# CoHDI/composable-resource-operator

Hardware: AMD Instinct MI355X
Metric: p50 GPU attach→CDI-ready latency (ms) + reconciles/sec at 1/2/4/8 MI355X (lower is better)
Workload: dtype bf16; 1 GPU; model=ComposabilityRequest(type=gpu, model=mi355x, size=1) bulk compose, global_batch=1, seq_len=0, fabric=mock (in-process; no physical CXL fabric on bench node), probe=True, force_detach=False, cpus=4, gc_frozen=True

## Files before the change

cro_amd/controllers/composableresource.py:

```python

from __future__ import annotations

import logging
import time
from dataclasses import dataclass
from typing import Dict, Optional

from ..api.v1alpha1.types import ComposableResource
from ..fabric import Adapter, FabricError, WaitingDeviceAttaching, WaitingDeviceDetaching
from ..metrics import Metrics
from ..nodeops import amdgpu, taints
from ..nodeops.amdgpu import GPULoadsPresent, ScrubFailed
from ..nodeops.nodes import node_exists
from ..runtime.client import Client
from ..runtime.controller import Reconciler, Result
from ..runtime.errors import ConflictError, NotFoundError
from ..runtime.store import _now_rfc3339

log = logging.getLogger(__name__)

FINALIZER = "cro.amd.com/finalizer"
READY_TO_DETACH_LABEL = "cro.amd.com/ready-to-detach-device-id"
READY_TO_DETACH_CDI_LABEL = "cro.amd.com/ready-to-detach-cdi-device-id"
MANAGED_BY_LABEL = "app.kubernetes.io/managed-by"
# ... 313 lines not shown
            for other in self.client.list(ComposableResource, copy=False):
                if (
                    other.metadata.name != resource.metadata.name
                    and other.status.device_id == device_id
                ):
                    raise FabricError(
                        f"fabric returned device {device_id} already claimed "
                        f"by {other.metadata.name}; refusing dual attachment"
                    )
            resource = self._persist_device_identity(
                resource.metadata.name, device_id, cdi_device_id
            )
            self._fabric_polls.pop(resource.metadata.uid, None)
            self.recorder.normal(
                resource, "FabricAttached", f"fabric composed device {device_id}"
            )

        if mode == "DEVICE_PLUGIN":
            try:
                ops.check_no_loads(node)
            except GPULoadsPresent as exc:
                log.warning("gpu loads during attach on %s: %s", node, exc)
            resource = self._restart_plugin_daemonsets(resource, fatal=False)
        with self._phase("node_refresh"):
            ops.refresh_after_attach(node)

        if mode == "DRA":
            visible = ops.is_visible_dra(node, resource.status.device_id)
        else:
            visible = ops.is_visible(node, resource.status.device_id)
        if not visible:
            return Result(requeue_after=self.config.attach_visible_wait)

        with self._phase("cdi_write"):
            ops.write_cdi(node, resource.status.device_id)
        with self._phase("health_probe"):
            probe = ops.health_probe(node, resource.status.device_id)
        if probe is not None and not probe.get("ok", True):
            compute = probe.get("compute")
            if isinstance(compute, dict) and not compute.get("ok", True):
                test = compute.get("failed_test") or (
                    "coverage" if compute.get("rc") == -31 else "unknown"
                )
                self.metrics.probe_compute_failures_total.labels(test=test).inc()
                raise FabricError(
                    "gfx950 health probe failed: compute stage "
# ... 239 lines not shown
```

cro_amd/hip/build.py:

```python

from __future__ import annotations

import os
import subprocess
import sys

HIP_DIR = os.path.dirname(os.path.abspath(__file__))
AGENT_DIR = os.path.join(os.path.dirname(HIP_DIR), "agent")
SRC = os.path.join(HIP_DIR, "probe.hip")
SRCS = [SRC, os.path.join(HIP_DIR, "integrity.hip")]
HEADERS = [os.path.join(HIP_DIR, "croprobe.h"), os.path.join(HIP_DIR, "cropattern.h")]
COVERAGE_SRC = os.path.join(HIP_DIR, "coverage.hip")
COVERAGE_HEADER = os.path.join(HIP_DIR, "crocoverage.h")
INTERNAL_HEADERS = [os.path.join(HIP_DIR, "crohost.h"), os.path.join(HIP_DIR, "cromfma.h")]
INTEGRITY_HEADER = os.path.join(HIP_DIR, "crointegrity.h")
ALL_SRCS = SRCS + [COVERAGE_SRC]
ALL_HEADERS = HEADERS + [COVERAGE_HEADER, INTEGRITY_HEADER] + INTERNAL_HEADERS
OUT = os.path.join(HIP_DIR, "libcroprobe.so")
SCRUB_SRC = os.path.join(HIP_DIR, "scrub.hip")
SCRUB_HEADERS = [
    os.path.join(HIP_DIR, "croscrub.h"),
    os.path.join(HIP_DIR, "croscrubplan.h"),
    os.path.join(HIP_DIR, "crohost.h"),
    INTEGRITY_HEADER,
    HEADERS[1],
]
SCRUB_OUT = os.path.join(HIP_DIR, "libcroscrub.so")
LDS_SCRUB_SRC = os.path.join(HIP_DIR, "ldsscrub.hip")
LDS_SCRUB_HEADERS = [
    os.path.join(HIP_DIR, "croldsscrub.h"),
    os.path.join(HIP_DIR, "crohost.h"),
    COVERAGE_HEADER,
]
LDS_SCRUB_OUT = os.path.join(HIP_DIR, "libcroldsscrub.so")
REG_SCRUB_SRC = os.path.join(HIP_DIR, "regscrub.hip")
REG_SCRUB_HEADERS = [
    os.path.join(HIP_DIR, "croregscrub.h"),
    os.path.join(HIP_DIR, "crohost.h"),
    COVERAGE_HEADER,
]
# ... 14 lines not shown
]
COHERENCE_OUT = os.path.join(HIP_DIR, "libcrocoherence.so")
MOVEMENT_SRC = os.path.join(HIP_DIR, "movement.hip")
MOVEMENT_HEADERS = [
    os.path.join(HIP_DIR, "cromovement.h"),
    os.path.join(HIP_DIR, "crohost.h"),
    COVERAGE_HEADER,
]
MOVEMENT_OUT = os.path.join(HIP_DIR, "libcromovement.so")
AGENT_SRC = os.path.join(AGENT_DIR, "croagent.cpp")
AGENT_OUT = os.path.join(AGENT_DIR, "croagent")
HIPCC = os.environ.get("HIPCC", "/opt/rocm/bin/hipcc")
DEVICE_FLAGS = ["--offload-arch=gfx950", "-O3"]


def _stale(out: str, inputs) -> bool:
    if not os.path.exists(out):
        return True
    built = os.path.getmtime(out)
    return any(os.path.getmtime(path) > built for path in inputs)


def build(force: bool = False) -> str:
    if force or _stale(OUT, ALL_SRCS + ALL_HEADERS):
        subprocess.run(
            [HIPCC, *DEVICE_FLAGS, "-fPIC", "-shared", *ALL_SRCS, "-o", OUT],
            check=True,
        )
    build_agent(force=force)
    return OUT


def build_scrub(force: bool = False) -> str:
    if force or _stale(SCRUB_OUT, [SCRUB_SRC] + SCRUB_HEADERS):
        subprocess.run(
            [HIPCC, *DEVICE_FLAGS, "-fPIC", "-shared", SCRUB_SRC, "-o", SCRUB_OUT],
            check=True,
        )
    return SCRUB_OUT


def build_lds_scrub(force: bool = False) -> str:
    if force or _stale(LDS_SCRUB_OUT, [LDS_SCRUB_SRC] + LDS_SCRUB_HEADERS):
        subprocess.run(
            [HIPCC, *DEVICE_FLAGS, "-fPIC", "-shared", LDS_SCRUB_SRC, "-o", LDS_SCRUB_OUT],
            check=True,
        )
# ... 71 lines not shown
```

cro_amd/hip/croprobe.h:

```cpp
#pragma once

#include "crocoverage.h"

#ifdef __cplusplus
extern "C" {
#endif

struct CroProbeResult {
  int ok;
  int mfma_f32_exact;
  double hbm_gbps;
  double bf16_tflops;
  long long vram_total;
  long long vram_free;
  double t_setup_ms;
  double t_mfma_ms;
  double t_bw_ms;
  double t_bf16_ms;
  char gcn_arch[64];
  char msg[256];
};

struct CroProbeOpts {
  double hbm_floor_gbps;
  double bf16_floor_tflops;
  int selftest_mode;
  int selftest_bit;
  unsigned int selftest_elem;
  int reserved;
};

int cro_probe_run(int device, struct CroProbeResult* out);
int cro_probe_run_opts(int device, const struct CroProbeOpts* opts, struct CroProbeResult* out);

struct CroProbeWindows {
  int copy_launches;
  int bf16_iters;
  int skip_check_launch;
  int reserved;
};

int cro_probe_run_windows(int device, const struct CroProbeWindows* w,
                          struct CroProbeResult* out);
int cro_probe_mfma_f32(int device, const float* A, const float* B, float* D, int K);
int cro_probe_copy(int device, const void* src_host, unsigned long long n4, int grid_blocks,
                   void* dst_host, int* guard_ok);
int cro_probe_bw_selfcheck(int device, unsigned long long* n_bad,
                           unsigned long long* first_bad);
int cro_probe_bf16_sink(int device, int blocks, int iters, int all_lanes, float* out_host);
void* cro_probe_alloc(int device, long long bytes);
void cro_probe_free(void* p);
int cro_probe_device_count(void);
int cro_probe_pci_bus_id(int device, char* buf, int len);


struct CroIntegrityOpts {
  long long vram_bytes;
  long long link_bytes;
  long long chunk_bytes;
  unsigned int seed;
  int selftest_stage;
  double link_floor_gbps;
  int selftest_pass;
  int selftest_bit;
  unsigned long long selftest_word;
};
// ... 99 lines not shown
```

cro_amd/hip/probe.hip:

```cpp

#include <hip/hip_runtime.h>
#include <hip/hip_bf16.h>
#include <cstring>
#include <vector>

#include "crohost.h"
#include "cromfma.h"
#include "croprobe.h"


__global__ void mfma_f32_check_kernel(const float* __restrict__ A,
                                      const float* __restrict__ B,
                                      float* __restrict__ D, int K) {
  const uint32_t lane = threadIdx.x;
  const f32x4 acc = wave_mfma_f32(A, B, K, lane);
  for (int r = 0; r < 4; ++r) D[mfma_elem16(lane, r)] = acc[r];
}


__global__ void bw_copy_kernel(const float4* __restrict__ src,
                               float4* __restrict__ dst, size_t n4) {
  size_t i = (size_t)blockIdx.x * blockDim.x + threadIdx.x;
  size_t stride = (size_t)gridDim.x * blockDim.x;
  for (; i < n4; i += stride) dst[i] = src[i];
}


template <bool kAllLanes>
__global__ void mfma_bf16_rate_kernel(float* __restrict__ out, int iters) {
  bf16x8 a, b;
  for (int i = 0; i < 8; ++i) {
// ... 9 lines not shown
  }
  float s = 0.f;
  for (int i = 0; i < 16; ++i) s += acc0[i] + acc1[i] + acc2[i] + acc3[i];
  if constexpr (kAllLanes) {
    out[blockIdx.x * 256 + threadIdx.x] = s;
  } else {
    if (threadIdx.x == 0) out[blockIdx.x] = s;
  }
}


enum { kEvCheck0, kEvCheck1, kEvCopies, kEvRate, kEvTile, kNumEvents };

struct ProbeCtx : CtxBase {
  long long vram_total = 0, vram_free = 0;
  float *dA = nullptr, *dB = nullptr, *dD = nullptr;
  float4 *src = nullptr, *dst = nullptr;
  float* sink = nullptr;
  hipStream_t stream = nullptr;
  hipEvent_t ev[kNumEvents] = {};
  float* hD = nullptr;
  float refD[CRO_COV_F32_ELEMS] = {0};
  char gcn_arch[64] = {0};
};
static ProbeCtx g_ctx[kMaxDevices];

constexpr int kBwGrid = 8192;
constexpr size_t kBwBytes = (size_t)256 << 20;
constexpr int kGuardVecs = 64;
constexpr unsigned long long kMaxCopyVecs = kBwBytes / sizeof(float4);
constexpr int kMaxCopyGrid = 1 << 16;
constexpr int kMaxSinkBlocks = 1024;
constexpr int kMaxSinkIters = 1 << 16;
constexpr int kRateBlocks = 1024;
constexpr int kDefaultCopyLaunches = 8;
constexpr int kDefaultBf16Iters = 1024;
constexpr int kMaxCopyLaunches = 64;
constexpr int kMaxBf16Iters = 1 << 16;

static void launch_copy(const float4* src, float4* dst, size_t n4, int grid_blocks,
                        hipStream_t stream = nullptr) {
  hipLaunchKernelGGL(bw_copy_kernel, dim3(grid_blocks), dim3(kBlock), 0, stream, src, dst, n4);
}

static void launch_probe_copy(const ProbeCtx* ctx) {
  launch_copy(ctx->src, ctx->dst, kBwBytes / sizeof(float4), kBwGrid, ctx->stream);
// ... 34 lines not shown
  ctx->vram_total = (long long)total_b;
  ctx->vram_free = (long long)free_b;
  TRY(hipDeviceSynchronize());
  TRY(hipMemsetAsync(ctx->dD, 0xFF, sizeof(ctx->refD), ctx->stream));
  launch_probe_check(ctx);
  launch_probe_copy(ctx);
  launch_probe_rate(ctx, 64);
  TRY(hipGetLastError());
  TRY(hipMemcpyAsync(ctx->hD, ctx->dD, sizeof(ctx->refD), hipMemcpyDeviceToHost, ctx->stream));
  TRY(hipStreamSynchronize(ctx->stream));
  ctx->ready = 1;
  return hipSuccess;
}

#define STEP(expr)                \
  do {                            \
    hipError_t _e = (expr);       \
    if (_e != hipSuccess) {       \
      *what = #expr;              \
      return _e;                  \
    }                             \
  } while (0)

static hipError_t enqueue_and_wait(ProbeCtx* ctx, int copy_launches, int bf16_iters,
                                   bool skip_check, bool* enqueued, const char** what) {
  hipStream_t st = ctx->stream;
  *enqueued = true;
  STEP(hipMemsetAsync(ctx->dD, 0xFF, sizeof(ctx->refD), st));
  STEP(hipEventRecord(ctx->ev[kEvCheck0], st));
  if (!skip_check) launch_probe_check(ctx);
  STEP(hipGetLastError());
  STEP(hipEventRecord(ctx->ev[kEvCheck1], st));
  for (int i = 0; i < copy_launches; ++i) launch_probe_copy(ctx);
  STEP(hipGetLastError());
  STEP(hipEventRecord(ctx->ev[kEvCopies], st));
  launch_probe_rate(ctx, bf16_iters);
  STEP(hipGetLastError());
  STEP(hipEventRecord(ctx->ev[kEvRate], st));
  STEP(hipMemcpyAsync(ctx->hD, ctx->dD, sizeof(ctx->refD), hipMemcpyDeviceToHost, st));
  STEP(hipEventRecord(ctx->ev[kEvTile], st));
  STEP(hipEventSynchronize(ctx->ev[kEvTile]));
  return hipSuccess;
}

#undef STEP

static int run_pipeline(int device, const struct CroProbeOpts& o, int copy_launches,
                        int bf16_iters, bool skip_check, struct CroProbeResult* out, double t0) {
  const double hbm_floor = o.hbm_floor_gbps > 0.0 ? o.hbm_floor_gbps : 500.0;
  const double bf16_floor = o.bf16_floor_tflops > 0.0 ? o.bf16_floor_tflops : 100.0;

  std::unique_lock<std::mutex> lock;
  ProbeCtx* ctx = enter_device(g_ctx, device, lock, out->msg, sizeof(out->msg));
  if (ctx == nullptr) return -1;
  CHECK(ensure_ctx(ctx, device));
  snprintf(out->gcn_arch, sizeof(out->gcn_arch), "%s", ctx->gcn_arch);
  out->vram_total = ctx->vram_total;
  out->vram_free = ctx->vram_free;
  out->t_setup_ms = now_ms() - t0;

  bool enqueued = false;
  const char* what = "";
  const hipError_t e = enqueue_and_wait(ctx, copy_launches, bf16_iters, skip_check, &enqueued,
                                        &what);
  if (e != hipSuccess) {
    if (enqueued) (void)hipStreamSynchronize(ctx->stream);
    snprintf(out->msg, sizeof(out->msg), "%s failed: %s", what, hipGetErrorString(e));
    return -1;
  }

  const float* want = ctx->refD;
  float flipped[CRO_COV_F32_ELEMS];
  if (o.selftest_mode == 1) {
    memcpy(flipped, ctx->refD, sizeof(flipped));
    uint32_t u;
    memcpy(&u, &flipped[o.selftest_elem], sizeof(u));
    u ^= 1u << o.selftest_bit;
    memcpy(&flipped[o.selftest_elem], &u, sizeof(u));
    want = flipped;
  }
  out->mfma_f32_exact = (memcmp(ctx->hD, want, sizeof(flipped)) == 0) ? 1 : 0;

  float ms = 0.f;
  CHECK(hipEventElapsedTime(&ms, ctx->ev[kEvCheck0], ctx->ev[kEvCheck1]));
  out->t_mfma_ms = ms;
  CHECK(hipEventElapsedTime(&ms, ctx->ev[kEvCheck1], ctx->ev[kEvCopies]));
  out->hbm_gbps = (double)(2.0 * kBwBytes * copy_launches) / (ms * 1e6);
  out->t_bw_ms = ms;
  CHECK(hipEventElapsedTime(&ms, ctx->ev[kEvCopies], ctx->ev[kEvRate]));
  double waves = (double)kRateBlocks * 256.0 / 64.0;
  double flops = waves * 4.0 * (double)bf16_iters * 2.0 * 32.0 * 32.0 * 16.0;
  out->bf16_tflops = flops / (ms * 1e9);
  out->t_bf16_ms = ms;

  if (!out->mfma_f32_exact) {
    snprintf(out->msg, sizeof(out->msg), "f32 MFMA mismatch vs host fmaf chain");
    return -2;
  }
  if (out->hbm_gbps < hbm_floor) {
    snprintf(out->msg, sizeof(out->msg), "HBM bandwidth %.0f GB/s below floor", out->hbm_gbps);
    return -3;
  }
  if (out->bf16_tflops < bf16_floor) {
    snprintf(out->msg, sizeof(out->msg), "bf16 MFMA %.0f TF below floor", out->bf16_tflops);
    return -4;
  }
  out->ok = 1;
  snprintf(out->msg, sizeof(out->msg), "ok");
  return 0;
}

extern "C" int cro_probe_run_opts(int device, const struct CroProbeOpts* opts,
                                  struct CroProbeResult* out) {
  memset(out, 0, sizeof(*out));
  out->ok = 0;
  const double t0 = now_ms();

  struct CroProbeOpts o;
  memset(&o, 0, sizeof(o));
  if (opts) o = *opts;
  if (!(o.hbm_floor_gbps >= 0.0)) return bad_arg(out, "hbm_floor_gbps");
  if (!(o.bf16_floor_tflops >= 0.0)) return bad_arg(out, "bf16_floor_tflops");
  if (o.selftest_mode < 0 || o.selftest_mode > 1) return bad_arg(out, "selftest_mode");
  if (o.selftest_bit < 0 || o.selftest_bit > 31) return bad_arg(out, "selftest_bit");
  if (o.selftest_elem >= CRO_COV_F32_ELEMS) return bad_arg(out, "selftest_elem");
  return run_pipeline(device, o, kDefaultCopyLaunches, kDefaultBf16Iters, false, out, t0);
}

extern "C" int cro_probe_run_windows(int device, const struct CroProbeWindows* w,
                                     struct CroProbeResult* out) {
  memset(out, 0, sizeof(*out));
  out->ok = 0;
  const double t0 = now_ms();

  struct CroProbeWindows win;
  memset(&win, 0, sizeof(win));
  if (w) win = *w;
  if (win.copy_launches < 0 || win.copy_launches > kMaxCopyLaunches)
    return bad_arg(out, "copy_launches");
  if (win.bf16_iters < 0 || win.bf16_iters > kMaxBf16Iters) return bad_arg(out, "bf16_iters");
  if (win.skip_check_launch < 0 || win.skip_check_launch > 1)
    return bad_arg(out, "skip_check_launch");
  if (win.reserved < 0) return bad_arg(out, "reserved");
  struct CroProbeOpts o;
  memset(&o, 0, sizeof(o));
  return run_pipeline(device, o, win.copy_launches ? win.copy_launches : kDefaultCopyLaunches,
                      win.bf16_iters ? win.bf16_iters : kDefaultBf16Iters,
                      win.skip_check_launch == 1, out, t0);
}

extern "C" int cro_probe_run(int device, struct CroProbeResult* out) {
  return cro_probe_run_opts(device, nullptr, out);
}


extern "C" int cro_probe_mfma_f32(int device, const float* A, const float* B,
                                  float* D, int K) {
  if (A == nullptr || B == nullptr || D == nullptr) return -10;
  if (K <= 0 || K > kMaxTileK || (K & 3) != 0) return -10;
  const size_t in_bytes = (size_t)16 * K * sizeof(float), out_bytes = 256 * sizeof(float);
  if (hipSetDevice(device) != hipSuccess) return -1;
  DevBuf<float> dA, dB, dD;
  const auto run = [&]() -> hipError_t {
    TRY(dA.alloc(in_bytes));
    TRY(dB.alloc(in_bytes));
    TRY(dD.alloc(out_bytes));
    TRY(hipMemcpy(dA.get(), A, in_bytes, hipMemcpyHostToDevice));
    TRY(hipMemcpy(dB.get(), B, in_bytes, hipMemcpyHostToDevice));
    hipLaunchKernelGGL(mfma_f32_check_kernel, dim3(1), dim3(64), 0, 0, dA.get(), dB.get(),
                       dD.get(), K);
    TRY(hipGetLastError());
// ... 19 lines not shown
    TRY(hipMemcpy(src.get(), src_host, bytes, hipMemcpyHostToDevice));
    TRY(hipMemset(dst.get(), 0xA5, bytes + guard_bytes));
    launch_copy(src.get(), dst.get(), (size_t)n4, grid_blocks);
    TRY(hipGetLastError());
    TRY(hipMemcpy(dst_host, dst.get(), bytes, hipMemcpyDeviceToHost));
    TRY(hipMemcpy(back.data(), dst.get() + n4, guard_bytes, hipMemcpyDeviceToHost));
    int ok = 1;
    for (size_t i = 0; i < guard_bytes; ++i) ok &= back[i] == 0xA5;
    *guard_ok = ok;
    return hipMemcpy(back.data(), src.get(), bytes, hipMemcpyDeviceToHost);
  };
  if (run() != hipSuccess) return -1;
  return memcmp(back.data(), src_host, bytes) == 0 ? 0 : -11;
}

extern "C" int cro_probe_bw_selfcheck(int device, unsigned long long* n_bad,
                                      unsigned long long* first_bad) {
  if (n_bad == nullptr || first_bad == nullptr) return -10;
  *n_bad = 0;
  *first_bad = ~0ull;
  std::unique_lock<std::mutex> lock;
  ProbeCtx* ctx = enter_device(g_ctx, device, lock, nullptr, 0);
  if (ctx == nullptr) return -1;
  const auto copy_once = [&]() -> hipError_t {
    TRY(ensure_ctx(ctx, device));
    TRY(hipMemsetAsync(ctx->dst, 0, kBwBytes, ctx->stream));
    launch_probe_copy(ctx);
    TRY(hipGetLastError());
    return hipSuccess;
  };
  const hipError_t enq = copy_once();
  const hipError_t done = ctx->stream ? hipStreamSynchronize(ctx->stream) : hipSuccess;
  if (enq != hipSuccess || done != hipSuccess) return -1;
  const size_t chunk = (size_t)32 << 20;
  std::vector<unsigned char> host(chunk);
  for (size_t off = 0; off < kBwBytes; off += chunk) {
    if (hipMemcpy(host.data(), (const unsigned char*)ctx->dst + off, chunk,
                  hipMemcpyDeviceToHost) != hipSuccess)
      return -1;
    for (size_t i = 0; i < chunk; i += 8) {
      unsigned long long w;
      memcpy(&w, &host[i], 8);
      if (w == 0x5a5a5a5a5a5a5a5aull) continue;
      for (size_t j = i; j < i + 8; ++j) {
        if (host[j] == 0x5a) continue;
        if (*n_bad == 0) *first_bad = off + j;
// ... 52 lines not shown
```

cro_amd/nodeops/amdgpu.py:

```python

from __future__ import annotations

import logging
import threading
import time
from typing import Callable, Dict, List, Optional, Set

from ..api.v1alpha1.types import ResourceSlice, ResourceSliceDevice, ResourceSliceSpec
from .cdi_spec import CDISpecWriter
from .execs import ExecError, NodeExec
from .kfd import GPUDevice, enumerate_gpus, enumerate_gpus_amdsmi, gpu_compute_pids

log = logging.getLogger(__name__)


class DriverMissing(Exception):
    pass


class GPULoadsPresent(Exception):
    pass


class ScrubFailed(Exception):
# ... 18 lines not shown

    def is_visible(self, node: str, device_id: str) -> bool:
        raise NotImplementedError

    def check_no_loads(self, node: str, device_id: Optional[str] = None) -> None:
        raise NotImplementedError

    def drain(self, node: str, device_id: str) -> None:
        raise NotImplementedError

    def refresh_after_attach(self, node: str) -> None:
        raise NotImplementedError

    def refresh_after_detach(self, node: str) -> None:
        raise NotImplementedError

    def write_cdi(self, node: str, device_id: str) -> str:
        raise NotImplementedError

    def remove_cdi(self, node: str, device_id: str) -> None:
        raise NotImplementedError

    def health_probe(self, node: str, device_id: str) -> Optional[dict]:
        return None

    def scrub(self, node: str, device_id: str) -> Optional[dict]:
        return None


class AmdNodeOps(NodeOps):
    def __init__(
        self,
        execer: NodeExec,
        client=None,
        cdi_dir: str = "/etc/cdi",
        destructive: bool = True,
        initially_detached: Optional[List[str]] = None,
        restart_hooks: Optional[Dict[str, Callable[[str], None]]] = None,
        probe_fn: Optional[Callable[[int], dict]] = None,
        publish_resource_slices: bool = True,
        scrub_fn: Optional[Callable[[GPUDevice], dict]] = None,
    ):
        self.execer = execer
        self.client = client
        self.cdi = CDISpecWriter(execer, cdi_dir)
        self.destructive = destructive
        self.publish_slices = publish_resource_slices
        self._sim_detached: Set[str] = set(initially_detached or [])
        self._sim_lock = threading.Lock()
        self.restart_hooks = restart_hooks or {}
        self.probe_fn = probe_fn
        self.scrub_fn = scrub_fn
        self._self_pid_cache: Dict[int, Optional[int]] = {}
        self._drain_lock = threading.Lock()
        self._drain_threads: Dict[str, threading.Thread] = {}
        self._drain_errors: Dict[str, str] = {}
        self.enum_cache_ttl = 0.025
        self._enum_cache: Dict[str, tuple] = {}
        self._enum_lock = threading.Lock()
        self._static_meta: dict = {}


    def driver_mode(self, node: str) -> str:
        if self.client is not None:
            from ..api.v1alpha1.types import DeviceConfig

            try:
                configs = self.client.list(DeviceConfig)
            except Exception:
                configs = []
            if any(dc.spec.driver.enable for dc in configs):
                return "container"
        if self.execer.path_exists(node, "/sys/module/amdgpu"):
            return "host"
        return "none"
# ... 149 lines not shown
            if cached is None and gpu_id not in self._self_pid_cache:
                hip_dev = None
                try:
                    from .probe import hip_device_for_bdf, load_library

                    if load_library(required=False) is not None:
                        for g in self.enumerate(node):
                            if g.gpu_id == gpu_id:
                                hip_dev = hip_device_for_bdf(g.pci_bdf)
                                break
                        if hip_dev is not None:
                            cached = resolve_self_kfd_pid(
                                self.execer, node, gpu_id, hip_dev
                            )
                except Exception as exc:
                    log.debug("self-pid resolution failed: %s", exc)
                self._self_pid_cache[gpu_id] = cached
            if cached is not None:
                own.add(cached)
        return own


    def drain(self, node: str, device_id: str) -> None:
        with self._drain_lock:
            thread = self._drain_threads.get(device_id)
            if thread is not None:
                if thread.is_alive():
                    raise DrainInProgress(f"drain of {device_id} still running")
                del self._drain_threads[device_id]
                err = self._drain_errors.pop(device_id, None)
                if err is not None:
                    raise ExecError(err)
                return

        gpu = self.find_gpu(node, device_id)
        if gpu is None:
            return
        if not self.destructive:
            with self._sim_lock:
                self._sim_detached.add(device_id)
            self._invalidate_enum(node)
            return
        remaining = [g for g in self.enumerate(node) if g.device_id != device_id]
        if remaining:
            self.execer.write_file(node, f"/sys/bus/pci/devices/{gpu.pci_bdf}/remove", "1")
            self._invalidate_enum(node)
# ... 4 lines not shown
        def unload_and_remove():
            try:
                rc, _, err = self.execer.run(node, modprobe_argv, timeout=120)
                if rc != 0:
                    raise ExecError(f"modprobe -r amdgpu failed: {err}", rc=rc, stderr=err)
                self.execer.write_file(
                    node, f"/sys/bus/pci/devices/{gpu.pci_bdf}/remove", "1"
                )
                self._invalidate_enum(node)
            except Exception as exc:
                with self._drain_lock:
                    self._drain_errors[device_id] = str(exc)

        t = threading.Thread(target=unload_and_remove, name=f"drain-{device_id}", daemon=True)
        with self._drain_lock:
            self._drain_threads[device_id] = t
        t.start()
        raise DrainInProgress(f"last-device drain of {device_id} started")

    def refresh_after_attach(self, node: str) -> None:
        if self.destructive:
            self.execer.write_file(node, "/sys/bus/pci/rescan", "1")
        self._invalidate_enum(node)
        for name, hook in self.restart_hooks.items():
            try:
                hook(node)
            except Exception as exc:
                log.warning("restart hook %s failed on %s: %s", name, node, exc)
        self._publish_slice(node)

    def simulate_compose(self, node: str, device_id: str) -> None:
        with self._sim_lock:
            self._sim_detached.discard(device_id)
        self._invalidate_enum(node)

    def refresh_after_detach(self, node: str) -> None:
        for name, hook in self.restart_hooks.items():
            try:
                hook(node)
            except Exception as exc:
                log.warning("restart hook %s failed on %s: %s", name, node, exc)
        self._publish_slice(node)

    def _publish_slice(self, node: str) -> None:
        if self.client is None or not self.publish_slices:
            return
        devices = [
            ResourceSliceDevice(
                name=f"gpu-{i}",
                uuid=g.device_id,
                model="mi355x",
                node=node,
# ... 13 lines not shown
            sl.spec = ResourceSliceSpec(node_name=node, pool=name, devices=devices)
            self.client.create(sl)
        else:
            existing.spec.devices = devices
            self.client.update(existing)


    def write_cdi(self, node: str, device_id: str) -> str:
        gpu = self.find_gpu(node, device_id)
        if gpu is None:
            raise ExecError(f"device {device_id} not enumerable; cannot write CDI spec")
        return self.cdi.add_device(node, gpu)

    def remove_cdi(self, node: str, device_id: str) -> None:
        self.cdi.remove_device(node, device_id)


    def health_probe(self, node: str, device_id: str) -> Optional[dict]:
        if self.probe_fn is None:
            return None
        gpu = self.find_gpu(node, device_id)
        if gpu is None:
            return None
        return self.probe_fn(gpu)

    def scrub(self, node: str, device_id: str) -> Optional[dict]:
        if self.scrub_fn is None:
            return None
        gpu = self.find_gpu(node, device_id)
        if gpu is None:
            return None
        return self.scrub_fn(gpu)


class MockNodeOps(NodeOps):

    def __init__(self, client=None, attach_visible_delay: float = 0.0):
        self.client = client
        self.driver_present: Dict[str, bool] = {}
        self.composed: Dict[str, Set[str]] = {}
        self.visible: Dict[str, Set[str]] = {}
        self.loads: Dict[str, Set[str]] = {}
        self.cdi_written: Dict[str, Set[str]] = {}
        from collections import deque

        self.calls: "deque[tuple]" = deque(maxlen=10000)
# ... 83 lines not shown
```

cro_amd/nodeops/probe.py:

```python

from __future__ import annotations

import ctypes
import os
from typing import Optional

_LIB_PATH = os.path.join(os.path.dirname(__file__), "..", "hip", "libcroprobe.so")


class CroProbeResult(ctypes.Structure):
    _fields_ = [
        ("ok", ctypes.c_int),
        ("mfma_f32_exact", ctypes.c_int),
        ("hbm_gbps", ctypes.c_double),
        ("bf16_tflops", ctypes.c_double),
        ("vram_total", ctypes.c_longlong),
        ("vram_free", ctypes.c_longlong),
        ("t_setup_ms", ctypes.c_double),
        ("t_mfma_ms", ctypes.c_double),
        ("t_bw_ms", ctypes.c_double),
        ("t_bf16_ms", ctypes.c_double),
        ("gcn_arch", ctypes.c_char * 64),
        ("msg", ctypes.c_char * 256),
    ]


class CroProbeOpts(ctypes.Structure):

# ... 156 lines not shown
    if _lib is not None:
        return _lib
    if required is None:
        required = _gpu_present()
    path = os.path.abspath(_LIB_PATH)
    if not os.path.exists(path):
        if required:
            raise RuntimeError(
                f"libcroprobe.so missing at {path} on a GPU node — build it with "
                "`python -m cro_amd.hip.build` (hipcc --offload-arch=gfx950)"
            )
        return None
    lib = ctypes.CDLL(path)
    lib.cro_probe_run.argtypes = [ctypes.c_int, ctypes.POINTER(CroProbeResult)]
    lib.cro_probe_run.restype = ctypes.c_int
    lib.cro_probe_run_opts.argtypes = [
        ctypes.c_int, ctypes.POINTER(CroProbeOpts), ctypes.POINTER(CroProbeResult),
    ]
    lib.cro_probe_run_opts.restype = ctypes.c_int
    lib.cro_probe_run_windows.argtypes = [
        ctypes.c_int, ctypes.POINTER(CroProbeWindows), ctypes.POINTER(CroProbeResult),
    ]
    lib.cro_probe_run_windows.restype = ctypes.c_int
    f32p = ctypes.POINTER(ctypes.c_float)
    lib.cro_probe_mfma_f32.argtypes = [ctypes.c_int, f32p, f32p, f32p, ctypes.c_int]
    lib.cro_probe_mfma_f32.restype = ctypes.c_int
    lib.cro_probe_copy.argtypes = [
        ctypes.c_int, ctypes.c_void_p, ctypes.c_ulonglong, ctypes.c_int, ctypes.c_void_p,
        ctypes.POINTER(ctypes.c_int),
    ]
    lib.cro_probe_copy.restype = ctypes.c_int
    lib.cro_probe_bw_selfcheck.argtypes = [
        ctypes.c_int, ctypes.POINTER(ctypes.c_ulonglong), ctypes.POINTER(ctypes.c_ulonglong),
    ]
    lib.cro_probe_bw_selfcheck.restype = ctypes.c_int
    lib.cro_probe_bf16_sink.argtypes = [
        ctypes.c_int, ctypes.c_int, ctypes.c_int, ctypes.c_int, ctypes.c_void_p,
    ]
    lib.cro_probe_bf16_sink.restype = ctypes.c_int
    lib.cro_probe_device_count.restype = ctypes.c_int
    lib.cro_probe_pci_bus_id.argtypes = [ctypes.c_int, ctypes.c_char_p, ctypes.c_int]
    lib.cro_probe_pci_bus_id.restype = ctypes.c_int
    lib.cro_probe_alloc.argtypes = [ctypes.c_int, ctypes.c_longlong]
    lib.cro_probe_alloc.restype = ctypes.c_void_p
    lib.cro_probe_free.argtypes = [ctypes.c_void_p]
    lib.cro_probe_free.restype = None
    lib.cro_probe_integrity.argtypes = [
# ... 107 lines not shown
def run_probe(device: int = 0, **opts) -> dict:
    lib = load_library(required=True)
    res = CroProbeResult()
    if opts:
        c_opts = _probe_opts(**opts)
        rc = lib.cro_probe_run_opts(device, ctypes.byref(c_opts), ctypes.byref(res))
    else:
        rc = lib.cro_probe_run(device, ctypes.byref(res))
    return _result_dict(res, rc)


def run_probe_windows(device: int = 0, copy_launches: int = 0, bf16_iters: int = 0,
                      skip_check_launch: int = 0) -> dict:
    lib = load_library(required=True)
    windows = CroProbeWindows(
        copy_launches=int(copy_launches), bf16_iters=int(bf16_iters),
        skip_check_launch=int(skip_check_launch),
    )
    res = CroProbeResult()
    rc = lib.cro_probe_run_windows(device, ctypes.byref(windows), ctypes.byref(res))
    return _result_dict(res, rc)


def probe_fn_for_nodeops(gpu) -> dict:
    dev = hip_device_for_bdf(gpu.pci_bdf)
    if dev is None:
        dev = 0
    return run_probe(dev)




def mfma_f32_tile(device: int, a, b):
    import numpy as np

    lib = load_library(required=True)
    a = np.ascontiguousarray(a, dtype=np.float32)
    b = np.ascontiguousarray(b, dtype=np.float32)
    k = a.shape[1] if a.ndim == 2 else -1
    if a.shape != (16, k) or b.shape != (k, 16):
        raise ValueError("f32 tile wants A 16xK and B Kx16")
    d = np.zeros((16, 16), dtype=np.float32)
    f32p = ctypes.POINTER(ctypes.c_float)
    rc = lib.cro_probe_mfma_f32(device, a.ctypes.data_as(f32p), b.ctypes.data_as(f32p),
                                d.ctypes.data_as(f32p), k)
    if rc != 0:
        raise RuntimeError(f"cro_probe_mfma_f32 failed: rc={rc}")
    return d


def copy_vectors(device: int, words, grid_blocks: int) -> dict:
# ... 409 lines not shown


def aggregate_records(records) -> dict:
    out, _, bad_keys = aggregate_wave_records(records, ("f32", "i8", "bf16", "lds"))
    out.update(n_bad_cu_keys=min(len(bad_keys), 8), bad_cu_keys=bad_keys[:8])
    return out


def make_probe_fn(level: str = "quick", vram_bytes: int = 0, link_bytes: int = 0,
                  link_floor_gbps: float = 0.0, seed: int = 0, compute: bool = False,
                  compute_min_cu_fraction: float = 0.0, formats: bool = False,
                  formats_min_cu_fraction: float = 0.0, coherence: bool = False,
                  coherence_min_cu_fraction: float = 0.0, movement: bool = False,
                  movement_min_cu_fraction: float = 0.0):
    if level not in PROBE_LEVELS:
        raise ValueError(f"unknown probe level {level!r} (expected one of {PROBE_LEVELS})")
    if level == "quick" and not compute and not formats and not coherence and not movement:
        return probe_fn_for_nodeops

    def staged_probe(gpu) -> dict:
        dev = hip_device_for_bdf(gpu.pci_bdf)
        if dev is None:
            dev = 0
        result = run_probe(dev)
        if not result.get("ok"):
            return result
        if compute:
            stage = run_compute(dev, seed=seed, min_cu_fraction=compute_min_cu_fraction)
            result["compute"] = stage
            if not stage.get("ok"):
                result["ok"] = False
                result["msg"] = stage.get("msg", "compute probe failed")
                return result
        if formats:
            from .formats import run_formats

            stage = run_formats(dev, seed=seed, min_cu_fraction=formats_min_cu_fraction)
            result["formats"] = stage
            if not stage.get("ok"):
                result["ok"] = False
                result["msg"] = stage.get("msg", "formats probe failed")
                return result
        if coherence:
            from .coherence import run_coherence

            stage = run_coherence(dev, seed=seed, min_cu_fraction=coherence_min_cu_fraction)
            result["coherence"] = stage
# ... 2 lines not shown
                result["msg"] = stage.get("msg", "coherence probe failed")
                return result
        if movement:
            from .movement import run_movement

            stage = run_movement(dev, seed=seed, min_cu_fraction=movement_min_cu_fraction)
            result["movement"] = stage
            if not stage.get("ok"):
                result["ok"] = False
                result["msg"] = stage.get("msg", "movement probe failed")
                return result
        if level == "deep":
            integrity = run_integrity(
                dev, vram_bytes=vram_bytes, link_bytes=link_bytes, seed=seed,
                link_floor_gbps=link_floor_gbps,
            )
            result["integrity"] = integrity
            if not integrity.get("ok"):
                result["ok"] = False
                result["msg"] = integrity.get("msg", "integrity probe failed")
        return result

    staged_probe.level = level
    staged_probe.compute = bool(compute)
    if formats:
        staged_probe.formats = True
    if coherence:
        staged_probe.coherence = True
    if movement:
        staged_probe.movement = True
    return staged_probe


def _compute_argv(compute, compute_min_cu_fraction) -> list:
    if not compute:
        return []
    argv = ["--compute"]
    if compute_min_cu_fraction:
        argv += ["--compute-min-cu-fraction", str(float(compute_min_cu_fraction))]
    return argv


def _formats_argv(formats, formats_min_cu_fraction) -> list:
    if not formats:
        return []
    argv = ["--formats"]
# ... 87 lines not shown
```

Baseline: 3.124 ms.

## Split GPU health probe into async submit/collect to overlap with node refresh

Adds a ticketed submit/collect/cancel API to the HIP probe library so the probe pipeline can be enqueued without waiting on its completion event. The controller now requests a probe before node refresh, nodeops submits it right after enumeration invalidation, and the later health_probe call collects the in-flight result instead of launching and synchronizing from scratch. This is meant to hide GPU probe execution behind node refresh, CDI write and the visibility check, at the cost of ticket bookkeeping, cancellation on drain, and a fallback to a synchronous run if the ticket is stale.

```diff
diff --git a/cro_amd/controllers/composableresource.py b/cro_amd/controllers/composableresource.py
--- a/cro_amd/controllers/composableresource.py
+++ b/cro_amd/controllers/composableresource.py
@@ -359,6 +359,9 @@
             except GPULoadsPresent as exc:
                 log.warning("gpu loads during attach on %s: %s", node, exc)
             resource = self._restart_plugin_daemonsets(resource, fatal=False)
+        begin_probe = getattr(ops, "begin_health_probe", None)
+        if begin_probe is not None:
+            begin_probe(node, resource.status.device_id)
         with self._phase("node_refresh"):
             ops.refresh_after_attach(node)
 
diff --git a/cro_amd/hip/build.py b/cro_amd/hip/build.py
--- a/cro_amd/hip/build.py
+++ b/cro_amd/hip/build.py
@@ -16,6 +16,7 @@
 INTEGRITY_HEADER = os.path.join(HIP_DIR, "crointegrity.h")
 ALL_SRCS = SRCS + [COVERAGE_SRC]
 ALL_HEADERS = HEADERS + [COVERAGE_HEADER, INTEGRITY_HEADER] + INTERNAL_HEADERS
+TICKETS_HEADER_NAME = "crotickets.h"
 OUT = os.path.join(HIP_DIR, "libcroprobe.so")
 SCRUB_SRC = os.path.join(HIP_DIR, "scrub.hip")
 SCRUB_HEADERS = [
@@ -76,7 +77,11 @@
 
 
 def build(force: bool = False) -> str:
-    if force or _stale(OUT, ALL_SRCS + ALL_HEADERS):
+    inputs = ALL_SRCS + ALL_HEADERS
+    tickets = os.path.join(os.path.dirname(HEADERS[0]), TICKETS_HEADER_NAME)
+    if os.path.exists(tickets):
+        inputs = inputs + [tickets]
+    if force or _stale(OUT, inputs):
         subprocess.run(
             [HIPCC, *DEVICE_FLAGS, "-fPIC", "-shared", *ALL_SRCS, "-o", OUT],
             check=True,
diff --git a/cro_amd/hip/croprobe.h b/cro_amd/hip/croprobe.h
--- a/cro_amd/hip/croprobe.h
+++ b/cro_amd/hip/croprobe.h
@@ -42,6 +42,12 @@
 
 int cro_probe_run_windows(int device, const struct CroProbeWindows* w,
                           struct CroProbeResult* out);
+
+int cro_probe_submit(int device, const struct CroProbeWindows* w, unsigned long long* ticket);
+#define CRO_PROBE_NOT_IN_FLIGHT (-5)
+int cro_probe_collect(int device, unsigned long long ticket, const struct CroProbeOpts* opts,
+                      struct CroProbeResult* out);
+int cro_probe_cancel(int device);
 int cro_probe_mfma_f32(int device, const float* A, const float* B, float* D, int K);
 int cro_probe_copy(int device, const void* src_host, unsigned long long n4, int grid_blocks,
                    void* dst_host, int* guard_ok);
diff --git a/cro_amd/hip/crotickets.h b/cro_amd/hip/crotickets.h
--- /dev/null
+++ b/cro_amd/hip/crotickets.h
@@ -0,0 +1,67 @@
+#pragma once
+
+#ifdef __cplusplus
+extern "C" {
+#endif
+
+enum CroTicketFate {
+  CRO_TICKET_IN_FLIGHT = 0,
+  CRO_TICKET_NEVER_ISSUED,
+  CRO_TICKET_COLLECTED,
+  CRO_TICKET_SUPERSEDED,
+  CRO_TICKET_CANCELLED,
+  CRO_TICKET_RETIRED,
+};
+
+enum { CRO_TICKET_HISTORY = 8 };
+
+struct CroTicketBook {
+  unsigned long long last_issued;
+  unsigned long long in_flight;
+  unsigned long long retired[CRO_TICKET_HISTORY];
+  int retired_fate[CRO_TICKET_HISTORY];
+  unsigned long long n_retired;
+};
+
+static inline unsigned long long cro_ticket_retire(struct CroTicketBook* b, int fate) {
+  const unsigned long long t = b->in_flight;
+  if (t == 0) return 0;
+  const unsigned long long slot = b->n_retired % CRO_TICKET_HISTORY;
+  b->retired[slot] = t;
+  b->retired_fate[slot] = fate;
+  ++b->n_retired;
+  b->in_flight = 0;
+  return t;
+}
+
+static inline unsigned long long cro_ticket_issue(struct CroTicketBook* b) {
+  (void)cro_ticket_retire(b, CRO_TICKET_SUPERSEDED);
+  if (++b->last_issued == 0) ++b->last_issued;
+  b->in_flight = b->last_issued;
+  return b->in_flight;
+}
+
+static inline int cro_ticket_match(const struct CroTicketBook* b, unsigned long long ticket) {
+  if (ticket != 0 && ticket == b->in_flight) return CRO_TICKET_IN_FLIGHT;
+  if (ticket == 0 || ticket > b->last_issued) return CRO_TICKET_NEVER_ISSUED;
+  const unsigned long long kept =
+      b->n_retired < CRO_TICKET_HISTORY ? b->n_retired : (unsigned long long)CRO_TICKET_HISTORY;
+  for (unsigned long long i = 0; i < kept; ++i)
+    if (b->retired[i] == ticket) return b->retired_fate[i];
+  return CRO_TICKET_RETIRED;
+}
+
+static inline const char* cro_ticket_fate_name(int fate) {
+  switch (fate) {
+    case CRO_TICKET_IN_FLIGHT: return "in flight";
+    case CRO_TICKET_NEVER_ISSUED: return "never issued";
+    case CRO_TICKET_COLLECTED: return "already collected";
+    case CRO_TICKET_SUPERSEDED: return "superseded";
+    case CRO_TICKET_CANCELLED: return "cancelled";
+    default: return "ended earlier";
+  }
+}
+
+#ifdef __cplusplus
+}
+#endif
diff --git a/cro_amd/hip/probe.hip b/cro_amd/hip/probe.hip
--- a/cro_amd/hip/probe.hip
+++ b/cro_amd/hip/probe.hip
@@ -7,6 +7,7 @@
 #include "crohost.h"
 #include "cromfma.h"
 #include "croprobe.h"
+#include "crotickets.h"
 
 
 __global__ void mfma_f32_check_kernel(const float* __restrict__ A,
@@ -62,6 +63,10 @@
   float* hD = nullptr;
   float refD[CRO_COV_F32_ELEMS] = {0};
   char gcn_arch[64] = {0};
+  CroTicketBook book = {};
+  int fl_copy_launches = 0, fl_bf16_iters = 0;
+  bool fl_skip_check = false;
+  double fl_setup_ms = 0.0;
 };
 static ProbeCtx g_ctx[kMaxDevices];
 
@@ -142,7 +147,7 @@
     }                             \
   } while (0)
 
-static hipError_t enqueue_and_wait(ProbeCtx* ctx, int copy_launches, int bf16_iters,
+static hipError_t enqueue_pipeline(ProbeCtx* ctx, int copy_launches, int bf16_iters,
                                    bool skip_check, bool* enqueued, const char** what) {
   hipStream_t st = ctx->stream;
   *enqueued = true;
@@ -159,35 +164,94 @@
   STEP(hipEventRecord(ctx->ev[kEvRate], st));
   STEP(hipMemcpyAsync(ctx->hD, ctx->dD, sizeof(ctx->refD), hipMemcpyDeviceToHost, st));
   STEP(hipEventRecord(ctx->ev[kEvTile], st));
-  STEP(hipEventSynchronize(ctx->ev[kEvTile]));
   return hipSuccess;
 }
 
 #undef STEP
 
-static int run_pipeline(int device, const struct CroProbeOpts& o, int copy_launches,
-                        int bf16_iters, bool skip_check, struct CroProbeResult* out, double t0) {
-  const double hbm_floor = o.hbm_floor_gbps > 0.0 ? o.hbm_floor_gbps : 500.0;
-  const double bf16_floor = o.bf16_floor_tflops > 0.0 ? o.bf16_floor_tflops : 100.0;
-
-  std::unique_lock<std::mutex> lock;
-  ProbeCtx* ctx = enter_device(g_ctx, device, lock, out->msg, sizeof(out->msg));
-  if (ctx == nullptr) return -1;
+static hipError_t end_in_flight(ProbeCtx* ctx, int fate) {
+  if (ctx->book.in_flight == 0) return hipSuccess;
+  const hipError_t e = hipStreamSynchronize(ctx->stream);
+  (void)cro_ticket_retire(&ctx->book, fate);
+  return e;
+}
+
+static int check_opts(const struct CroProbeOpts* opts, struct CroProbeOpts* o,
+                      struct CroProbeResult* out) {
+  memset(o, 0, sizeof(*o));
+  if (opts) *o = *opts;
+  if (!(o->hbm_floor_gbps >= 0.0)) return bad_arg(out, "hbm_floor_gbps");
+  if (!(o->bf16_floor_tflops >= 0.0)) return bad_arg(out, "bf16_floor_tflops");
+  if (o->selftest_mode < 0 || o->selftest_mode > 1) return bad_arg(out, "selftest_mode");
+  if (o->selftest_bit < 0 || o->selftest_bit > 31) return bad_arg(out, "selftest_bit");
+  if (o->selftest_elem >= CRO_COV_F32_ELEMS) return bad_arg(out, "selftest_elem");
+  return 0;
+}
+
+static int check_windows(const struct CroProbeWindows* w, struct CroProbeWindows* win,
+                         struct CroProbeResult* out) {
+  memset(win, 0, sizeof(*win));
+  if (w) *win = *w;
+  if (win->copy_launches < 0 || win->copy_launches > kMaxCopyLaunches)
+    return bad_arg(out, "copy_launches");
+  if (win->bf16_iters < 0 || win->bf16_iters > kMaxBf16Iters) return bad_arg(out, "bf16_iters");
+  if (win->skip_check_launch < 0 || win->skip_check_launch > 1)
+    return bad_arg(out, "skip_check_launch");
+  if (win->reserved < 0) return bad_arg(out, "reserved");
+  if (win->copy_launches == 0) win->copy_launches = kDefaultCopyLaunches;
+  if (win->bf16_iters == 0) win->bf16_iters = kDefaultBf16Iters;
+  return 0;
+}
+
+static int submit_locked(ProbeCtx* ctx, int device, const struct CroProbeWindows& win, double t0,
+                         unsigned long long* ticket, struct CroProbeResult* out) {
+  *ticket = 0;
+  CHECK(end_in_flight(ctx, CRO_TICKET_SUPERSEDED));
   CHECK(ensure_ctx(ctx, device));
-  snprintf(out->gcn_arch, sizeof(out->gcn_arch), "%s", ctx->gcn_arch);
-  out->vram_total = ctx->vram_total;
-  out->vram_free = ctx->vram_free;
-  out->t_setup_ms = now_ms() - t0;
+  const double setup_ms = now_ms() - t0;
 
   bool enqueued = false;
   const char* what = "";
-  const hipError_t e = enqueue_and_wait(ctx, copy_launches, bf16_iters, skip_check, &enqueued,
-                                        &what);
+  const hipError_t e = enqueue_pipeline(ctx, win.copy_launches, win.bf16_iters,
+                                        win.skip_check_launch == 1, &enqueued, &what);
   if (e != hipSuccess) {
     if (enqueued) (void)hipStreamSynchronize(ctx->stream);
     snprintf(out->msg, sizeof(out->msg), "%s failed: %s", what, hipGetErrorString(e));
     return -1;
   }
+  ctx->fl_copy_launches = win.copy_launches;
+  ctx->fl_bf16_iters = win.bf16_iters;
+  ctx->fl_skip_check = win.skip_check_launch == 1;
+  ctx->fl_setup_ms = setup_ms;
+  *ticket = cro_ticket_issue(&ctx->book);
+  return 0;
+}
+
+static int collect_locked(ProbeCtx* ctx, unsigned long long ticket, const struct CroProbeOpts& o,
+                          struct CroProbeResult* out) {
+  const int fate = cro_ticket_match(&ctx->book, ticket);
+  if (fate != CRO_TICKET_IN_FLIGHT) {
+    snprintf(out->msg, sizeof(out->msg), "ticket %llu is not in flight: %s", ticket,
+             cro_ticket_fate_name(fate));
+    return CRO_PROBE_NOT_IN_FLIGHT;
+  }
+  const double hbm_floor = o.hbm_floor_gbps > 0.0 ? o.hbm_floor_gbps : 500.0;
+  const double bf16_floor = o.bf16_floor_tflops > 0.0 ? o.bf16_floor_tflops : 100.0;
+  const int copy_launches = ctx->fl_copy_launches, bf16_iters = ctx->fl_bf16_iters;
+  snprintf(out->gcn_arch, sizeof(out->gcn_arch), "%s", ctx->gcn_arch);
+  out->vram_total = ctx->vram_total;
+  out->vram_free = ctx->vram_free;
+  out->t_setup_ms = ctx->fl_setup_ms;
+
+  const hipError_t e = hipEventSynchronize(ctx->ev[kEvTile]);
+  if (e != hipSuccess) {
+    (void)hipStreamSynchronize(ctx->stream);
+    (void)cro_ticket_retire(&ctx->book, CRO_TICKET_COLLECTED);
+    snprintf(out->msg, sizeof(out->msg), "hipEventSynchronize(ctx->ev[kEvTile]) failed: %s",
+             hipGetErrorString(e));
+    return -1;
+  }
+  (void)cro_ticket_retire(&ctx->book, CRO_TICKET_COLLECTED);
 
   const float* want = ctx->refD;
   float flipped[CRO_COV_F32_ELEMS];
@@ -230,21 +294,27 @@
   return 0;
 }
 
+static int run_pipeline(int device, const struct CroProbeOpts& o, const struct CroProbeWindows& win,
+                        struct CroProbeResult* out, double t0) {
+  std::unique_lock<std::mutex> lock;
+  ProbeCtx* ctx = enter_device(g_ctx, device, lock, out->msg, sizeof(out->msg));
+  if (ctx == nullptr) return -1;
+  unsigned long long ticket = 0;
+  const int rc = submit_locked(ctx, device, win, t0, &ticket, out);
+  if (rc != 0) return rc;
+  return collect_locked(ctx, ticket, o, out);
+}
+
 extern "C" int cro_probe_run_opts(int device, const struct CroProbeOpts* opts,
                                   struct CroProbeResult* out) {
   memset(out, 0, sizeof(*out));
   out->ok = 0;
   const double t0 = now_ms();
-
   struct CroProbeOpts o;
-  memset(&o, 0, sizeof(o));
-  if (opts) o = *opts;
-  if (!(o.hbm_floor_gbps >= 0.0)) return bad_arg(out, "hbm_floor_gbps");
-  if (!(o.bf16_floor_tflops >= 0.0)) return bad_arg(out, "bf16_floor_tflops");
-  if (o.selftest_mode < 0 || o.selftest_mode > 1) return bad_arg(out, "selftest_mode");
-  if (o.selftest_bit < 0 || o.selftest_bit > 31) return bad_arg(out, "selftest_bit");
-  if (o.selftest_elem >= CRO_COV_F32_ELEMS) return bad_arg(out, "selftest_elem");
-  return run_pipeline(device, o, kDefaultCopyLaunches, kDefaultBf16Iters, false, out, t0);
+  struct CroProbeWindows win;
+  if (check_opts(opts, &o, out) != 0) return -1;
+  if (check_windows(nullptr, &win, out) != 0) return -1;
+  return run_pipeline(device, o, win, out, t0);
 }
 
 extern "C" int cro_probe_run_windows(int device, const struct CroProbeWindows* w,
@@ -252,21 +322,45 @@
   memset(out, 0, sizeof(*out));
   out->ok = 0;
   const double t0 = now_ms();
-
+  struct CroProbeOpts o;
   struct CroProbeWindows win;
-  memset(&win, 0, sizeof(win));
-  if (w) win = *w;
-  if (win.copy_launches < 0 || win.copy_launches > kMaxCopyLaunches)
-    return bad_arg(out, "copy_launches");
-  if (win.bf16_iters < 0 || win.bf16_iters > kMaxBf16Iters) return bad_arg(out, "bf16_iters");
-  if (win.skip_check_launch < 0 || win.skip_check_launch > 1)
-    return bad_arg(out, "skip_check_launch");
-  if (win.reserved < 0) return bad_arg(out, "reserved");
+  if (check_windows(w, &win, out) != 0) return -1;
+  if (check_opts(nullptr, &o, out) != 0) return -1;
+  return run_pipeline(device, o, win, out, t0);
+}
+
+extern "C" int cro_probe_submit(int device, const struct CroProbeWindows* w,
+                                unsigned long long* ticket) {
+  if (ticket == nullptr) return -1;
+  *ticket = 0;
+  const double t0 = now_ms();
+  struct CroProbeResult scratch;
+  memset(&scratch, 0, sizeof(scratch));
+  struct CroProbeWindows win;
+  if (check_windows(w, &win, &scratch) != 0) return -1;
+  std::unique_lock<std::mutex> lock;
+  ProbeCtx* ctx = enter_device(g_ctx, device, lock, scratch.msg, sizeof(scratch.msg));
+  if (ctx == nullptr) return -1;
+  return submit_locked(ctx, device, win, t0, ticket, &scratch);
+}
+
+extern "C" int cro_probe_collect(int device, unsigned long long ticket,
+                                 const struct CroProbeOpts* opts, struct CroProbeResult* out) {
+  memset(out, 0, sizeof(*out));
+  out->ok = 0;
   struct CroProbeOpts o;
-  memset(&o, 0, sizeof(o));
-  return run_pipeline(device, o, win.copy_launches ? win.copy_launches : kDefaultCopyLaunches,
-                      win.bf16_iters ? win.bf16_iters : kDefaultBf16Iters,
-                      win.skip_check_launch == 1, out, t0);
+  if (check_opts(opts, &o, out) != 0) return -1;
+  std::unique_lock<std::mutex> lock;
+  ProbeCtx* ctx = enter_device(g_ctx, device, lock, out->msg, sizeof(out->msg));
+  if (ctx == nullptr) return -1;
+  return collect_locked(ctx, ticket, o, out);
+}
+
+extern "C" int cro_probe_cancel(int device) {
+  std::unique_lock<std::mutex> lock;
+  ProbeCtx* ctx = enter_device(g_ctx, device, lock, nullptr, 0);
+  if (ctx == nullptr) return -1;
+  return end_in_flight(ctx, CRO_TICKET_CANCELLED) == hipSuccess ? 0 : -1;
 }
 
 extern "C" int cro_probe_run(int device, struct CroProbeResult* out) {
@@ -332,6 +426,7 @@
   std::unique_lock<std::mutex> lock;
   ProbeCtx* ctx = enter_device(g_ctx, device, lock, nullptr, 0);
   if (ctx == nullptr) return -1;
+  if (end_in_flight(ctx, CRO_TICKET_SUPERSEDED) != hipSuccess) return -1;
   const auto copy_once = [&]() -> hipError_t {
     TRY(ensure_ctx(ctx, device));
     TRY(hipMemsetAsync(ctx->dst, 0, kBwBytes, ctx->stream));
diff --git a/cro_amd/nodeops/amdgpu.py b/cro_amd/nodeops/amdgpu.py
--- a/cro_amd/nodeops/amdgpu.py
+++ b/cro_amd/nodeops/amdgpu.py
@@ -64,6 +64,9 @@
         raise NotImplementedError
 
     def health_probe(self, node: str, device_id: str) -> Optional[dict]:
+        return None
+
+    def begin_health_probe(self, node: str, device_id: str) -> None:
         return None
 
     def scrub(self, node: str, device_id: str) -> Optional[dict]:
@@ -82,6 +85,7 @@
         probe_fn: Optional[Callable[[int], dict]] = None,
         publish_resource_slices: bool = True,
         scrub_fn: Optional[Callable[[GPUDevice], dict]] = None,
+        probe_begin_fn: Optional[Callable[[GPUDevice], None]] = None,
     ):
         self.execer = execer
         self.client = client
@@ -93,6 +97,13 @@
         self.restart_hooks = restart_hooks or {}
         self.probe_fn = probe_fn
         self.scrub_fn = scrub_fn
+        if probe_begin_fn is None:
+            probe_begin_fn = getattr(probe_fn, "begin", None)
+        self.probe_begin_fn = probe_begin_fn
+        self._probe_cancel_fn = getattr(probe_begin_fn, "cancel", None)
+        self._probe_lock = threading.Lock()
+        self._probe_wanted: Dict[str, Set[str]] = {}
+        self._probe_begun: Dict[str, GPUDevice] = {}
         self._self_pid_cache: Dict[int, Optional[int]] = {}
         self._drain_lock = threading.Lock()
         self._drain_threads: Dict[str, threading.Thread] = {}
@@ -288,6 +299,7 @@
 
 
     def drain(self, node: str, device_id: str) -> None:
+        self._cancel_begun_probe(node, device_id)
         with self._drain_lock:
             thread = self._drain_threads.get(device_id)
             if thread is not None:
@@ -338,12 +350,48 @@
         if self.destructive:
             self.execer.write_file(node, "/sys/bus/pci/rescan", "1")
         self._invalidate_enum(node)
+        self._begin_wanted_probes(node)
         for name, hook in self.restart_hooks.items():
             try:
                 hook(node)
             except Exception as exc:
                 log.warning("restart hook %s failed on %s: %s", name, node, exc)
         self._publish_slice(node)
+
+    def begin_health_probe(self, node: str, device_id: str) -> None:
+        if self.probe_fn is None or self.probe_begin_fn is None:
+            return
+        with self._probe_lock:
+            self._probe_wanted.setdefault(node, set()).add(device_id)
+
+    def _begin_wanted_probes(self, node: str) -> None:
+        with self._probe_lock:
+            wanted = self._probe_wanted.pop(node, None)
+        if not wanted:
+            return
+        for gpu in self.enumerate(node):
+            if gpu.device_id not in wanted:
+                continue
+            try:
+                self.probe_begin_fn(gpu)
+            except Exception as exc:
+                log.warning("probe begin for %s failed on %s: %s", gpu.device_id, node, exc)
+                continue
+            with self._probe_lock:
+                self._probe_begun[gpu.device_id] = gpu
+
+    def _cancel_begun_probe(self, node: str, device_id: str) -> None:
+        with self._probe_lock:
+            wanted = self._probe_wanted.get(node)
+            if wanted:
+                wanted.discard(device_id)
+            gpu = self._probe_begun.pop(device_id, None)
+        if gpu is None or self._probe_cancel_fn is None:
+            return
+        try:
+            self._probe_cancel_fn(gpu)
+        except Exception as exc:
+            log.warning("probe cancel for %s failed on %s: %s", device_id, node, exc)
 
     def simulate_compose(self, node: str, device_id: str) -> None:
         with self._sim_lock:
@@ -403,6 +451,8 @@
         gpu = self.find_gpu(node, device_id)
         if gpu is None:
             return None
+        with self._probe_lock:
+            self._probe_begun.pop(device_id, None)
         return self.probe_fn(gpu)
 
     def scrub(self, node: str, device_id: str) -> Optional[dict]:
diff --git a/cro_amd/nodeops/probe.py b/cro_amd/nodeops/probe.py
--- a/cro_amd/nodeops/probe.py
+++ b/cro_amd/nodeops/probe.py
@@ -2,8 +2,12 @@
 from __future__ import annotations
 
 import ctypes
+import logging
 import os
+import threading
 from typing import Optional
+
+log = logging.getLogger(__name__)
 
 _LIB_PATH = os.path.join(os.path.dirname(__file__), "..", "hip", "libcroprobe.so")
 
@@ -206,7 +210,18 @@
         ctypes.c_int, ctypes.POINTER(CroProbeWindows), ctypes.POINTER(CroProbeResult),
     ]
     lib.cro_probe_run_windows.restype = ctypes.c_int
-    f32p = ctypes.POINTER(ctypes.c_float)
+    lib.cro_probe_submit.argtypes = [
+        ctypes.c_int, ctypes.POINTER(CroProbeWindows), ctypes.POINTER(ctypes.c_ulonglong),
+    ]
+    lib.cro_probe_submit.restype = ctypes.c_int
+    lib.cro_probe_collect.argtypes = [
+        ctypes.c_int, ctypes.c_ulonglong, ctypes.POINTER(CroProbeOpts),
+        ctypes.POINTER(CroProbeResult),
+    ]
+    lib.cro_probe_collect.restype = ctypes.c_int
+    lib.cro_probe_cancel.argtypes = [ctypes.c_int]
+    lib.cro_probe_cancel.restype = ctypes.c_int
+    f32p =ctypes.POINTER(ctypes.c_float)
     lib.cro_probe_mfma_f32.argtypes = [ctypes.c_int, f32p, f32p, f32p, ctypes.c_int]
     lib.cro_probe_mfma_f32.restype = ctypes.c_int
     lib.cro_probe_copy.argtypes = [
@@ -360,11 +375,81 @@
     return _result_dict(res, rc)
 
 
+PROBE_NOT_IN_FLIGHT = -5
+
+
+def submit_probe(device: int = 0, copy_launches: int = 0, bf16_iters: int = 0,
+                 skip_check_launch: int = 0):
+    lib = load_library(required=True)
+    ticket = ctypes.c_ulonglong(0)
+    windows = None
+    if copy_launches or bf16_iters or skip_check_launch:
+        windows = ctypes.byref(CroProbeWindows(
+            copy_launches=int(copy_launches), bf16_iters=int(bf16_iters),
+            skip_check_launch=int(skip_check_launch),
+        ))
+    rc = lib.cro_probe_submit(device, windows, ctypes.byref(ticket))
+    return rc, ticket.value
+
+
+def collect_probe(device: int, ticket: int, **opts) -> dict:
+    lib = load_library(required=True)
+    res = CroProbeResult()
+    c_opts = ctypes.byref(_probe_opts(**opts)) if opts else None
+    rc = lib.cro_probe_collect(device, int(ticket), c_opts, ctypes.byref(res))
+    return _result_dict(res, rc)
+
+
+def cancel_probe(device: int = 0) -> int:
+    return load_library(required=True).cro_probe_cancel(device)
+
+
+_pending_lock = threading.Lock()
+_pending_tickets: dict = {}
+
+
+def _ordinal(gpu) -> int:
+    dev = hip_device_for_bdf(gpu.pci_bdf)
+    return 0 if dev is None else dev
+
+
+def begin_probe_for_nodeops(gpu) -> None:
+    dev = _ordinal(gpu)
+    rc, ticket = submit_probe(dev)
+    with _pending_lock:
+        if rc == 0:
+            _pending_tickets[dev] = ticket
+        else:
+            _pending_tickets.pop(dev, None)
+    if rc != 0:
+        log.warning("probe submit on HIP device %d failed (rc=%d); probing synchronously", dev, rc)
+
+
+def cancel_probe_for_nodeops(gpu) -> None:
+    dev = _ordinal(gpu)
+    with _pending_lock:
+        _pending_tickets.pop(dev, None)
+    cancel_probe(dev)
+
+
+begin_probe_for_nodeops.cancel = cancel_probe_for_nodeops
+
+
+def _collect_or_run(dev: int) -> dict:
+    with _pending_lock:
+        ticket = _pending_tickets.pop(dev, None)
+    if ticket:
+        result = collect_probe(dev, ticket)
+        if result["rc"] != PROBE_NOT_IN_FLIGHT:
+            return result
+    return run_probe(dev)
+
+
 def probe_fn_for_nodeops(gpu) -> dict:
-    dev = hip_device_for_bdf(gpu.pci_bdf)
-    if dev is None:
-        dev = 0
-    return run_probe(dev)
+    return _collect_or_run(_ordinal(gpu))
+
+
+probe_fn_for_nodeops.begin = begin_probe_for_nodeops
 
 
 
@@ -820,7 +905,7 @@
         dev = hip_device_for_bdf(gpu.pci_bdf)
         if dev is None:
             dev = 0
-        result = run_probe(dev)
+        result = _collect_or_run(dev)
         if not result.get("ok"):
             return result
         if compute:
@@ -869,6 +954,7 @@
         return result
 
     staged_probe.level = level
+    staged_probe.begin = begin_probe_for_nodeops
     staged_probe.compute = bool(compute)
     if formats:
         staged_probe.formats = True
```

Measured after the change: 3.166 ms. 1.3% more time.
